# davidcotton/gym-d2d

Hardware: AMD Instinct MI355X
Metric: env agent-steps/sec (batch x agents) (higher is better)
Workload: dtype f32

## Files before the change

### gym_d2d_amd/csrc/d2d_capi.hip

```cpp
#include "../../include/d2d_hip_diag.h"
#include "d2d_internal.h"
#include "d2d_plan.h"

#include <dlfcn.h>

#include <algorithm>
#include <cmath>
#include <cstdio>
#include <cstdlib>
#include <cstring>
#include <exception>
#include <new>
#include <stdexcept>
#include <string>
#include <vector>

namespace {

thread_local std::string g_last_error;

int fail(int code, const std::string& msg) {
    g_last_error = msg;
    return code;
}
// ... 743 lines not shown
        h->table_per_env = 1;
        h->table_links = n_links;
        h->mode = d2d::PL_TABLE_DB;
        h->have_pl = true; h->tables_dirty = true;
        return D2D_OK;
    }
    const size_t elems = (size_t)n_links * n_links * (per_env ? (size_t)h->B : 1);
    int rc = reserve_gain_table(h, elems);
    if (rc) return rc;
    HIP_TRY(d2d::launch_gain_from_db(pl_db_dev, dtype == D2D_F64, elems, h->gain_table, h->num_cus, h->stream));
    HIP_TRY(hipStreamSynchronize(h->stream));
    h->table_per_env = per_env ? 1 : 0;
    h->table_links = n_links;
    h->mode = d2d::PL_TABLE;
    h->have_pl = true; h->tables_dirty = true;
    return D2D_OK;
} D2D_CATCH

int d2d_set_path_loss_link_table(d2d_handle* h, const double* pl_db, int32_t n_links, int32_t per_env) try {
    if (!h || !pl_db) return fail(D2D_ERR_INVALID, "null argument");
    USE_DEVICE(h);
    if (!h->have_links) return fail(D2D_ERR_STATE, "d2d_set_links first: the table is indexed by its link list");
    if (n_links != h->N || n_links < 1) return fail(D2D_ERR_INVALID, "n_links must be the length of the current link list (" + std::to_string(h->N) + ")");
    const size_t elems = (size_t)n_links * n_links * (per_env ? (size_t)h->B : 1);
    int rc = upload_gain_table(h, pl_db, elems);
    if (rc) return rc;
    h->table_per_env = per_env ? 1 : 0;
    h->table_links = n_links;
    h->mode = d2d::PL_TABLE;
    h->have_pl = true; h->tables_dirty = true;
    return D2D_OK;
} D2D_CATCH

int d2d_set_links(d2d_handle* h, int32_t n_links, const int32_t* tx_dev, const int32_t* rx_dev, const int32_t* link_type) try {
    if (!h) return fail(D2D_ERR_INVALID, "null handle");
    USE_DEVICE(h);
    if (n_links < 0 || n_links > h->Nmax) return fail(D2D_ERR_INVALID, "n_links must be in [0, max_links]");
    if (n_links > 0 && (!tx_dev || !rx_dev || !link_type)) return fail(D2D_ERR_INVALID, "null argument");
    for (int i = 0; i < n_links; ++i) {
        if (tx_dev[i] < 0 || tx_dev[i] >= h->D || rx_dev[i] < 0 || rx_dev[i] >= h->D)
            return fail(D2D_ERR_INVALID, "link " + std::to_string(i) + ": device index out of range");
        if (link_type[i] < D2D_UPLINK || link_type[i] > D2D_SIDELINK)
            return fail(D2D_ERR_INVALID, "link " + std::to_string(i) + ": link_type must be 1, 2 or 3");
    }
    HIP_TRY(hipStreamSynchronize(h->stream));
    h->N = n_links;
    h->host_tx.assign(tx_dev, tx_dev + n_links);
    h->host_rx.assign(rx_dev, rx_dev + n_links);
    h->host_type.assign(link_type, link_type + n_links);
    h->fixed_rb.assign((size_t)n_links, INT32_MIN);
    h->fixed_pwr.assign((size_t)n_links, 0);
    h->n_fixed = 0;
    h->tables_dirty = true;
    h->lpos_dirty = true;
    h->have_links = true;
    if (h->table_links) {
        h->table_links = 0;
        h->live_table = nullptr;
        if (d2d::pl_is_table(h->mode)) h->have_pl = false;
    }
    return D2D_OK;
} D2D_CATCH

int d2d_set_fixed_actions(d2d_handle* h, int32_t n_fixed, const int32_t* link_idx, const int32_t* rb, const int32_t* pwr_dbm) try {
    if (!h) return fail(D2D_ERR_INVALID, "null handle");
    if (!h->have_links) return fail(D2D_ERR_STATE, "d2d_set_links first: fixed actions refer to its link list");
    if (n_fixed < 0 || n_fixed > h->N) return fail(D2D_ERR_INVALID, "n_fixed must be in [0, n_links]");
    if (n_fixed > 0 && (!link_idx || !rb || !pwr_dbm)) return fail(D2D_ERR_INVALID, "null argument");
    std::vector<int> frb((size_t)h->N, INT32_MIN), fpw((size_t)h->N, 0);
    for (int k = 0; k < n_fixed; ++k) {
        const int i = link_idx[k];
        if (i < 0 || i >= h->N) return fail(D2D_ERR_INVALID, "fixed action " + std::to_string(k) + ": link index out of range");
        if (frb[i] != INT32_MIN) return fail(D2D_ERR_INVALID, "fixed action " + std::to_string(k) + ": link listed twice");
        if (rb[k] == INT32_MIN) return fail(D2D_ERR_INVALID, "rb out of range");
        frb[i] = rb[k]; fpw[i] = pwr_dbm[k];
    }
    h->fixed_rb.swap(frb); h->fixed_pwr.swap(fpw);
    h->n_fixed = n_fixed;
    h->tables_dirty = true;
    return D2D_OK;
} D2D_CATCH

int d2d_positions_changed(d2d_handle* h) try {
    if (!h) return fail(D2D_ERR_INVALID, "null handle");
    h->lpos_dirty = true;
    h->have_lo = false;
    return D2D_OK;
} D2D_CATCH

int d2d_set_reward(d2d_handle* h, int32_t reward_fn, float param) try {
    if (!h) return fail(D2D_ERR_INVALID, "null handle");
    USE_DEVICE(h);
    if (reward_fn < D2D_REWARD_NONE || reward_fn > D2D_REWARD_CUE_SINR_SHANNON) return fail(D2D_ERR_INVALID, "unknown reward_fn");
    h->reward_fn = reward_fn; h->reward_param = param;
    return D2D_OK;
} D2D_CATCH

int d2d_set_reward_layout(d2d_handle* h, int32_t layout) try {
    if (!h) return fail(D2D_ERR_INVALID, "null handle");
    if (layout != D2D_REWARD_PER_AGENT && layout != D2D_REWARD_PER_ENV) return fail(D2D_ERR_INVALID, "unknown reward layout");
    h->reward_layout = layout;
    return D2D_OK;
} D2D_CATCH

int d2d_set_obs_dtype(d2d_handle* h, int32_t dtype) try {
    if (!h) return fail(D2D_ERR_INVALID, "null handle");
    if (dtype != D2D_F32 && dtype != D2D_F64) return fail(D2D_ERR_INVALID, "obs dtype must be D2D_F32 or D2D_F64");
    USE_DEVICE(h);
    if ((dtype == D2D_F64) != (h->obs_f64 != 0)) {
        Buffer& bf = h->buf[D2D_BUF_OBS];
        if (bf.ptr && bf.owned) { HIP_TRY(hipStreamSynchronize(h->stream)); HIP_TRY(hipFree(bf.ptr)); bf.ptr = nullptr; bf.bytes = 0; }
    }
    h->obs_f64 = dtype == D2D_F64;
    return D2D_OK;
} D2D_CATCH

int d2d_set_obs_mode(d2d_handle* h, int32_t obs_mode) try {
    if (!h) return fail(D2D_ERR_INVALID, "null handle");
    USE_DEVICE(h);
    if (obs_mode < D2D_OBS_NONE || obs_mode > D2D_OBS_LINEAR) return fail(D2D_ERR_INVALID, "unknown obs_mode");
    h->obs_mode = obs_mode;
    return D2D_OK;
} D2D_CATCH

int d2d_set_export_actions(d2d_handle* h, int32_t enabled) try {
    if (!h) return fail(D2D_ERR_INVALID, "null handle");
    h->export_actions = enabled ? 1 : 0;
    return D2D_OK;
} D2D_CATCH

int d2d_set_bucketing(d2d_handle* h, int32_t enabled) try {
    if (!h) return fail(D2D_ERR_INVALID, "null handle");
    USE_DEVICE(h);
    h->bucketing = enabled ? 1 : 0;
    return D2D_OK;
} D2D_CATCH

#if defined(D2D_STEP_ABLATE) && D2D_STEP_ABLATE
extern "C" int d2d_debug_stamps(d2d_handle* h, void* host, size_t bytes) try {
    if (!h || !h->dbg) return fail(D2D_ERR_STATE, "no stamps: set D2D_TUNE_STEP_ABLATE bit 8192 and step first");
    USE_DEVICE(h);
    HIP_TRY(hipStreamSynchronize(h->stream));
    if (!host || bytes > (size_t)h->B * 16 * 16 * 8) return fail(D2D_ERR_INVALID, "stamps: at most B x 16 waves x 16 stamps x 8 bytes");
    HIP_TRY(hipMemcpy(host, h->dbg, bytes, hipMemcpyDeviceToHost));
    return D2D_OK;
} D2D_CATCH
#endif

int d2d_set_tuning(d2d_handle* h, int32_t key, int32_t value) try {
    if (!h) return fail(D2D_ERR_INVALID, "null handle");
    USE_DEVICE(h);
#if !(defined(D2D_DIAG) && D2D_DIAG)
    const bool diag_key = key == D2D_TUNE_OBS_VARIANT || key == D2D_TUNE_OBS_STAGGER || key == D2D_TUNE_STEP_ABLATE;
    const bool diag_value = (key == D2D_TUNE_OBS_NONTEMPORAL && value > 1) || (key == D2D_TUNE_STEP_WALK && value == 1);
    if ((diag_key && value != 0) || diag_value)
        return fail(D2D_ERR_UNSUPPORTED, "this tuning key / value needs the diagnostic build (D2D_BUILD_DIAG=1 python -m gym_d2d_amd.build; include/d2d_hip_diag.h)");
#endif
    switch (key) {
        case D2D_TUNE_OBS_ROWS_PER_WG: h->tune_obs.rows = value; break;
        case D2D_TUNE_OBS_NONTEMPORAL:
            if (value < 0 || value > 5) return fail(D2D_ERR_INVALID, "obs store policy must be in [0, 5]");
            h->tune_obs.nt = value;
            break;
        case D2D_TUNE_OBS_XCD_REMAP: h->tune_obs.xcd = value < 0 ? 0 : value; break;
        case D2D_TUNE_OBS_VARIANT: h->tune_obs.variant = value; break;
        case D2D_TUNE_OBS_STAGGER:
            if (value < 0 || value > 64) return fail(D2D_ERR_INVALID, "stagger must be in [0, 64]");
            h->tune_obs.stagger = value;
            break;
        case D2D_TUNE_STEP_THREADS:
            if (value != 0 && (value < 64 || value > 1024 || value % 64)) return fail(D2D_ERR_INVALID, "threads must be a multiple of 64 in [64,1024]");
            h->tune_step.threads = value;
            break;
        case D2D_TUNE_OBS_BLOCK:
            if (value != 0 && (value < 64 || value > 1024 || value % 64)) return fail(D2D_ERR_INVALID, "block must be a multiple of 64 in [64,1024]");
            h->tune_obs.block = value;
            break;
        case D2D_TUNE_STEP_ENVS_PER_WG:
            if (value < 0 || value > 16) return fail(D2D_ERR_INVALID, "envs per workgroup must be in [0,16]");
            h->tune_step.epw = value;
            break;
        case D2D_TUNE_STEP_BLOCK:
            if (value != 0 && (value < 64 || value > 1024 || value % 64)) return fail(D2D_ERR_INVALID, "block must be a multiple of 64 in [64,1024]");
            h->tune_step.block = value;
            break;
        case D2D_TUNE_STEP_PREFETCH:
            if (value < -1) return fail(D2D_ERR_INVALID, "prefetch distance must be >= -1");
            h->tune_step.prefetch = value;
            break;
        case D2D_TUNE_STEP_LPT:
            if (value != -1 && value != 1 && value != 2) return fail(D2D_ERR_INVALID, "links per thread must be -1 (auto), 1 or 2");
            h->tune_step.lpt = value;
            break;
        case D2D_TUNE_STEP_WALK:
            if (value < -1 || value > 2) return fail(D2D_ERR_INVALID, "walk must be -1, 0, 1 or 2");
            h->tune_step.walk = value;
            break;
        case D2D_TUNE_STEP_ABLATE:
#if defined(D2D_STEP_ABLATE) && D2D_STEP_ABLATE
            h->tune_step.ablate = value;
            break;
#else
            if (value != 0) return fail(D2D_ERR_UNSUPPORTED, "D2D_TUNE_STEP_ABLATE needs the diagnostic build (D2D_BUILD_DIAG=1 python -m gym_d2d_amd.build)");
            break;
#endif
        case D2D_TUNE_STEP_OBS_ROTATE:
            if (value < -1 || value > 65535) return fail(D2D_ERR_INVALID, "obs_rotate must be in [-1, 65535]");
            h->tune_step.obs_rotate = value;
            break;
        case D2D_TUNE_STEP_NT_RESULTS:
            if (value < -1 || value > 1) return fail(D2D_ERR_INVALID, "nt_results must be -1, 0 or 1");
            h->tune_step.nt = value;
            break;
        case D2D_TUNE_STEP_SCALAR_RECORDS:
            if (value < -1 || value > 1) return fail(D2D_ERR_INVALID, "scalar_records must be -1, 0 or 1");
            h->tune_step.srec = value;
            break;
        case D2D_TUNE_STEP_FUSE_OBS:
            if (value < -1 || value > 1) return fail(D2D_ERR_INVALID, "fuse_obs must be -1, 0 or 1");
            h->tune_step.fuse = value;
            break;
        default: return fail(D2D_ERR_INVALID, "unknown tuning key");
    }
    return D2D_OK;
} D2D_CATCH

int d2d_get_buffer(d2d_handle* h, int32_t which, void** dev_ptr, size_t* bytes) try {
    if (!h || !dev_ptr) return fail(D2D_ERR_INVALID, "null argument");
    USE_DEVICE(h);
    if (which < 0 || which >= D2D_BUF_COUNT) return fail(D2D_ERR_INVALID, "unknown buffer");
    if (which == D2D_BUF_OBS && h->N == 0) return fail(D2D_ERR_STATE, "set links before asking for the obs buffer");
    int rc;
    if (which == D2D_BUF_LINK_POS) {
        if (!h->have_links || !h->have_pos) return fail(D2D_ERR_STATE, "link positions need d2d_set_links and positions first");
        rc = refresh_tables(h);
        if (rc) return rc;
        void *px = nullptr, *py = nullptr;
        rc = ensure_buffer(h, D2D_BUF_POS_X, &px);
        if (rc) return rc;
        rc = ensure_buffer(h, D2D_BUF_POS_Y, &py);
        if (rc) return rc;
        rc = refresh_link_positions(h, static_cast<const float*>(px), static_cast<const float*>(py));
        if (rc) return rc;
    }
    rc = ensure_buffer(h, which, dev_ptr);
    if (rc) return rc;
    if (bytes) *bytes = active_bytes(h, which, h->N ? h->N : h->Nmax);
    return D2D_OK;
} D2D_CATCH

int d2d_bind_buffer(d2d_handle* h, int32_t which, void* dev_ptr, size_t bytes) try {
    if (!h) return fail(D2D_ERR_INVALID, "null handle");
    USE_DEVICE(h);
    if (which < 0 || which >= D2D_BUF_COUNT) return fail(D2D_ERR_INVALID, "unknown buffer");
    if (which == D2D_BUF_LINK_POS) return fail(D2D_ERR_INVALID, "D2D_BUF_LINK_POS is derived from POS_X / POS_Y by the library: read-only");
    Buffer& bf = h->buf[which];
    HIP_TRY(hipStreamSynchronize(h->stream));
    if (bf.ptr && bf.owned) HIP_TRY(hipFree(bf.ptr));
    bf.ptr = dev_ptr; bf.bytes = dev_ptr ? bytes : 0; bf.owned = false;
    if (which == D2D_BUF_POS_X || which == D2D_BUF_POS_Y) {
        h->have_pos = h->buf[D2D_BUF_POS_X].ptr && h->buf[D2D_BUF_POS_Y].ptr;
        h->lpos_dirty = true;
        h->have_lo = false;
    }
    return D2D_OK;
} D2D_CATCH

int d2d_upload(d2d_handle* h, int32_t which, const void* host_src, size_t bytes, size_t dst_offset) try {
    if (!h || !host_src) return fail(D2D_ERR_INVALID, "null argument");
    USE_DEVICE(h);
    if (which < 0 || which >= D2D_BUF_COUNT) return fail(D2D_ERR_INVALID, "unknown buffer");
    if (which == D2D_BUF_LINK_POS) return fail(D2D_ERR_INVALID, "D2D_BUF_LINK_POS is derived from POS_X / POS_Y by the library: read-only");
    void* p = nullptr;
    int rc = ensure_buffer(h, which, &p);
    if (rc) return rc;
    if (dst_offset + bytes > h->buf[which].bytes) return fail(D2D_ERR_INVALID, "upload out of range");
    HIP_TRY(hipMemcpyAsync(static_cast<char*>(p) + dst_offset, host_src, bytes, hipMemcpyHostToDevice, h->stream));
    HIP_TRY(hipStreamSynchronize(h->stream));
    if (which == D2D_BUF_POS_X || which == D2D_BUF_POS_Y) {
        h->have_pos = h->buf[D2D_BUF_POS_X].ptr && h->buf[D2D_BUF_POS_Y].ptr;
        h->lpos_dirty = true;
        h->have_lo = false;
    }
    return D2D_OK;
} D2D_CATCH

int d2d_download(d2d_handle* h, int32_t which, void* host_dst, size_t bytes, size_t src_offset) try {
    if (!h || !host_dst) return fail(D2D_ERR_INVALID, "null argument");
    USE_DEVICE(h);
    if (which < 0 || which >= D2D_BUF_COUNT) return fail(D2D_ERR_INVALID, "unknown buffer");
    Buffer bf = h->buf[which];
    if (which == D2D_BUF_LINK_POS) {
        size_t n = 0;
        int rc = d2d_get_buffer(h, which, &bf.ptr, &n);
        if (rc) return rc;
        bf.bytes = n;
    }
    if (!bf.ptr) return fail(D2D_ERR_STATE, "buffer has never been written");
    if (src_offset + bytes > bf.bytes) return fail(D2D_ERR_INVALID, "download out of range");
    HIP_TRY(hipMemcpyAsync(host_dst, static_cast<const char*>(bf.ptr) + src_offset, bytes, hipMemcpyDeviceToHost, h->stream));
    HIP_TRY(hipStreamSynchronize(h->stream));
    return D2D_OK;
} D2D_CATCH

int d2d_set_positions(d2d_handle* h, const float* x, const float* y, int32_t env_begin, int32_t env_count) try {
    if (!h || !x || !y) return fail(D2D_ERR_INVALID, "null argument");
    if (env_begin < 0 || env_count < 0 || env_begin + env_count > h->B) return fail(D2D_ERR_INVALID, "env range out of bounds");
    const size_t off = (size_t)env_begin * h->D * 4, bytes = (size_t)env_count * h->D * 4;
    const bool keep_lo = h->have_lo && env_count < h->B;
    int rc = d2d_upload(h, D2D_BUF_POS_X, x, bytes, off);
    if (rc) return rc;
    rc = d2d_upload(h, D2D_BUF_POS_Y, y, bytes, off);
    if (rc) return rc;
    if (keep_lo) {
// ... 294 lines not shown
```

### gym_d2d_amd/csrc/d2d_internal.h

```cpp
#pragma once
#include <hip/hip_runtime.h>
#include <stdint.h>

namespace d2d {

enum PlMode : int {
    PL_INV_SQUARE = 0,
    PL_POWER = 1,
    PL_TABLE = 2,
    PL_SHADOW = 3,
    PL_POWK = 4,
    PL_TABLE_DB = 5
};

__host__ __device__ constexpr bool pl_is_table(int mode) { return mode == PL_TABLE || mode == PL_TABLE_DB; }

#define D2D_REC_TXDEV_MASK 0x00FFFFFF
#define D2D_REC_TYPE_SHIFT 24
#define D2D_REC_TYPE_MASK 0xF
#define D2D_REC_FIXED_BIT (1 << 28)

#define OPT_LISTS 1
#define OPT_SREC 2
#define OPT_NT 4
#define OPT_PAD 8
#define OPT_XPOS 16

#define LDS_HEAD_BYTES 80u
struct StepLds {
    unsigned aux, rx, sinr, sh, expo, tflat, mask, lists, pool, env_bytes;
    unsigned lo;
};

struct StepArgs {
    int B, N, R, D;
    int mask_words;
    int lpt;
    int rollout;
    StepLds lds;
    int action_mode;
    int act_stride;
    int col_mode;
    int n_fixed;
    int tpe;
    unsigned tpe_magic;
    float inv_n;
    int epw;
    int prefetch_envs;
    int walk;
    int reward_fn;
    float reward_param;
    int write_table;
    int pow_k;
    int rec_uniform;
    int nt_results;
    int ablate;
    unsigned long long* dbg;
    int fuse_obs;
    int obs_rotate;
    unsigned obs_q_per_row;
    unsigned long long obs_q_magic;
    const int* actions;
    const int* rb_in;
    const int* pwr_in;
    const int4* rec_a;
    const float4* rec_b;
    const float4* rec_c;
    const float2* rec_h;
    const int* rec_grp;
    const int* act_cols;
    const unsigned* side_words;
    const float4* lpos;
    const float4* lpos_lo;
    const float* gain_table;
    long long table_env_stride;
    int table_by_link;
    int table_pitch;
    float shadow_chi;
    float shadow_d0sq;
    unsigned shadow_seed_lo, shadow_seed_hi, shadow_step;
    unsigned long long env_offset;
    int* rb_out;
    int* pwr_out;
    float* sinr_db;
    float* snr_db;
    float* rate;
    float* cap;
    float* reward;
    float* reward_env;
    float* table;
    float* obs;
    int* env_flags;
};

struct ObsArgs {
    int B, N;
    int rows_per_wg;
    int chunks;
    int vec;
    unsigned q_per_row;
    unsigned long long q_magic;
    int xcd_remap;
    int nontemporal;
    int block;
    int variant;
    int out_f64;
    int stagger;
    const float* table;
    float* obs;
};

struct StepPlan;
hipError_t launch_step(const StepArgs& a, const StepPlan& p, hipStream_t stream);
hipError_t launch_rollout(const StepArgs& a, const StepPlan& p, hipStream_t stream);
hipError_t launch_obs_expand(const ObsArgs& a, hipStream_t stream);
hipError_t launch_flags_or(const int* env_flags, int B, unsigned* status, hipStream_t stream);
hipError_t launch_link_positions(const float* pos_x, const float* pos_y, const float* lo_x, const float* lo_y, const int4* rec_a,
                                 int B, int N, int D, float4* lpos, float4* lpos_lo, hipStream_t stream);
hipError_t launch_gain_from_db(const void* pl_db, int is_f64, size_t elems, float* gain, int num_cus, hipStream_t stream);
hipError_t launch_reset(int B, int D, int C, float cell_radius, float d2d_radius, unsigned long long seed,
                        unsigned long long episode, unsigned long long env_offset, const unsigned char* fixed_mask,
                        const float* fixed_xy, float* pos_x, float* pos_y, float4* lpos, int N, hipStream_t stream);
hipError_t launch_reset_masked(int B, int D, int C, float cell_radius, float d2d_radius, unsigned long long seed,
                               unsigned long long env_offset, const unsigned char* fixed_mask, const float* fixed_xy, float* pos_x,
                               float* pos_y, float4* lpos, int N, const int* pending, const unsigned* episode, float* lo_x, float* lo_y,
                               const int4* rec_a, float4* rows, float4* rows_lo, hipStream_t stream);

}
```

### gym_d2d_amd/csrc/d2d_obs.hip

```cpp
#include "d2d_internal.h"
#include "d2d_store.h"

namespace d2d {

__device__ __forceinline__ unsigned src_col(unsigned f, unsigned i) {
    const unsigned head = 6u * i;
    return f < 6u ? head + f : (f < head + 6u ? f - 6u : f);
}

template <int VEC, int NT>
__global__ __launch_bounds__(1024) void obs_expand_kernel(const ObsArgs a) {
    extern __shared__ __align__(16) float t_flat[];
    const unsigned N = a.N, tid = threadIdx.x, T = blockDim.x;
    unsigned env, chunk;
    if (a.xcd_remap) {
        const unsigned bid = blockIdx.x, lane8 = bid & 7u, rest = bid >> 3, G = (unsigned)a.xcd_remap;
        const unsigned per_group = a.chunks * G, group = rest / per_group, within = rest % per_group;
        chunk = within / G;
        env = (group * G + within % G) * 8u + lane8;
    } else {
        env = blockIdx.x / a.chunks;
        chunk = blockIdx.x % a.chunks;
    }
    const unsigned row_floats = 6u * N;

    {
        const f32x2* src = reinterpret_cast<const f32x2*>(a.table + (size_t)env * row_floats);
        f32x2* dst = reinterpret_cast<f32x2*>(t_flat);
        for (unsigned k = tid; k < row_floats / 2; k += T) dst[k] = src[k];
    }
    __syncthreads();

    const unsigned r0 = chunk * a.rows_per_wg;
    const unsigned r1 = min(r0 + (unsigned)a.rows_per_wg, N);
    const unsigned q_per_row = a.q_per_row;
    const unsigned total = (r1 - r0) * q_per_row;
    float* out = a.obs + ((size_t)env * N + r0) * row_floats;
    if (a.stagger > 0) {
        const int n = (int)(tid >> 6) * a.stagger;
        for (int k = 0; k < n; ++k) __builtin_amdgcn_s_sleep(1);
    }

    if (VEC == 4 && q_per_row == T) {
        const unsigned f0 = tid * 4u, f1 = f0 + 2u;
        const unsigned t0 = f0 / 6u, t1 = f1 / 6u;
        const bool own0 = f0 < 6u, own1 = f1 < 6u;
        f32x4* o4 = reinterpret_cast<f32x4*>(out) + tid;
        const f32x2* t2 = reinterpret_cast<const f32x2*>(t_flat);
        const auto row = [&](unsigned i) {
            const unsigned head = 6u * i;
            const unsigned s0 = own0 ? head + f0 : (i >= t0 ? f0 - 6u : f0);
            const unsigned s1 = own1 ? head + f1 : (i >= t1 ? f1 - 6u : f1);
            const f32x2 lo = t2[s0 >> 1], hi = t2[s1 >> 1];
            const f32x4 v = {lo.x, lo.y, hi.x, hi.y};
            return v;
        };
        unsigned i = r0;
        for (; i + 1u < r1; i += 2u) {
            const f32x4 va = row(i), vb = row(i + 1u);
            store16<NT>(o4 + (size_t)(i - r0) * T, va);
            store16<NT>(o4 + (size_t)(i + 1u - r0) * T, vb);
        }
        if (i < r1) store16<NT>(o4 + (size_t)(i - r0) * T, row(i));
        return;
    }
#pragma unroll 4
    for (unsigned idx = tid; idx < total; idx += T) {
        const unsigned lr = (unsigned)(((unsigned long long)idx * a.q_magic) >> 40);
        const unsigned q = idx - lr * q_per_row;
        const unsigned i = r0 + lr;
        const unsigned f = q * VEC;
        if (VEC == 4) {
            const f32x2 lo = reinterpret_cast<const f32x2*>(t_flat)[src_col(f, i) >> 1];
            const f32x2 hi = reinterpret_cast<const f32x2*>(t_flat)[src_col(f + 2u, i) >> 1];
            const f32x4 v = {lo.x, lo.y, hi.x, hi.y};
            store16<NT>(reinterpret_cast<f32x4*>(out + (size_t)idx * 4), v);
        } else {
            const f32x2 v = reinterpret_cast<const f32x2*>(t_flat)[src_col(f, i) >> 1];
            f32x2* p = reinterpret_cast<f32x2*>(out + (size_t)idx * 2);
            if (NT) __builtin_nontemporal_store(v, p); else *p = v;
        }
    }
}

template <int NT>
__global__ __launch_bounds__(1024) void obs_expand_flat_kernel(const ObsArgs a) {
    extern __shared__ __align__(16) float t_flat[];
    const unsigned N = a.N, tid = threadIdx.x, T = blockDim.x;
    unsigned env, chunk;
    if (a.xcd_remap) {
        const unsigned bid = blockIdx.x, lane8 = bid & 7u, rest = bid >> 3;
        chunk = rest % a.chunks; env = (rest / a.chunks) * 8u + lane8;
    } else {
        env = blockIdx.x / a.chunks; chunk = blockIdx.x % a.chunks;
    }
    const unsigned row_floats = 6u * N, q_per_row = a.q_per_row, total = N * q_per_row;
    {
        const f32x2* src = reinterpret_cast<const f32x2*>(a.table + (size_t)env * row_floats);
        f32x2* dst = reinterpret_cast<f32x2*>(t_flat);
        for (unsigned k = tid; k < row_floats / 2; k += T) dst[k] = src[k];
    }
    __syncthreads();
    if (a.stagger > 0) {
        const int n = (int)(tid >> 6) * a.stagger;
        for (int k = 0; k < n; ++k) __builtin_amdgcn_s_sleep(1);
    }
    const f32x2* t2 = reinterpret_cast<const f32x2*>(t_flat);
    f32x4* out = reinterpret_cast<f32x4*>(a.obs + (size_t)env * N * row_floats);
    const unsigned base = chunk * (unsigned)a.rows_per_wg * T;
    f32x4 v[4];
    unsigned idx[4];
#pragma unroll
    for (int p = 0; p < 4; ++p) {
        idx[p] = base + (unsigned)p * T + tid;
        if (p < a.rows_per_wg && idx[p] < total) {
            const unsigned i = (unsigned)(((unsigned long long)idx[p] * a.q_magic) >> 40), q = idx[p] - i * q_per_row;
            const unsigned f = q * 4u;
            const f32x2 lo = t2[src_col(f, i) >> 1], hi = t2[src_col(f + 2u, i) >> 1];
            v[p] = f32x4{lo.x, lo.y, hi.x, hi.y};
        }
    }
#pragma unroll
    for (int p = 0; p < 4; ++p)
        if (p < a.rows_per_wg && idx[p] < total) store16<NT>(out + idx[p], v[p]);
}

template <bool NT>
__global__ __launch_bounds__(1024) void obs_expand_f64_kernel(const ObsArgs a) {
    extern __shared__ __align__(16) float t_flat[];
    typedef double f64x2 __attribute__((ext_vector_type(2)));
    const unsigned N = a.N, tid = threadIdx.x, T = blockDim.x;
    unsigned env, chunk;
    if (a.xcd_remap) {
        const unsigned bid = blockIdx.x, lane8 = bid & 7u, rest = bid >> 3, G = (unsigned)a.xcd_remap;
        const unsigned per_group = a.chunks * G, group = rest / per_group, within = rest % per_group;
        chunk = within / G;
        env = (group * G + within % G) * 8u + lane8;
    } else {
        env = blockIdx.x / a.chunks;
        chunk = blockIdx.x % a.chunks;
    }
    const unsigned row_floats = 6u * N, q2 = row_floats / 2u;
    {
        const f32x2* src = reinterpret_cast<const f32x2*>(a.table + (size_t)env * row_floats);
        f32x2* dst = reinterpret_cast<f32x2*>(t_flat);
        for (unsigned k = tid; k < q2; k += T) dst[k] = src[k];
    }
    __syncthreads();
    const unsigned r0 = chunk * a.rows_per_wg;
    const unsigned r1 = min(r0 + (unsigned)a.rows_per_wg, N);
    const f32x2* t2 = reinterpret_cast<const f32x2*>(t_flat);
    double* out = reinterpret_cast<double*>(a.obs) + ((size_t)env * N + r0) * row_floats;
    for (unsigned i = r0; i < r1; ++i) {
        const unsigned head = 6u * i;
        f64x2* o = reinterpret_cast<f64x2*>(out + (size_t)(i - r0) * row_floats);
#pragma unroll 2
        for (unsigned c = tid; c < q2; c += T) {
            const unsigned f = 2u * c;
            const f32x2 v = t2[src_col(f, i) >> 1];
            const f64x2 d = {(double)v.x, (double)v.y};
            if (NT) __builtin_nontemporal_store(d, o + c); else o[c] = d;
        }
        (void)head;
    }
}

template <int NT>
__global__ __launch_bounds__(1024) void obs_expand_flat_f64_kernel(const ObsArgs a) {
    extern __shared__ __align__(16) float t_flat[];
    typedef double f64x2 __attribute__((ext_vector_type(2)));
    const unsigned N = a.N, tid = threadIdx.x, T = blockDim.x;
    unsigned env, chunk;
    if (a.xcd_remap) {
        const unsigned bid = blockIdx.x, lane8 = bid & 7u, rest = bid >> 3;
        chunk = rest % a.chunks; env = (rest / a.chunks) * 8u + lane8;
    } else {
        env = blockIdx.x / a.chunks; chunk = blockIdx.x % a.chunks;
    }
    const unsigned row_floats = 6u * N, q_per_row = a.q_per_row, total = N * q_per_row;
    {
        const f32x2* src = reinterpret_cast<const f32x2*>(a.table + (size_t)env * row_floats);
        f32x2* dst = reinterpret_cast<f32x2*>(t_flat);
        for (unsigned k = tid; k < row_floats / 2; k += T) dst[k] = src[k];
    }
    __syncthreads();
    const f32x2* t2 = reinterpret_cast<const f32x2*>(t_flat);
    f64x2* out = reinterpret_cast<f64x2*>(reinterpret_cast<double*>(a.obs) + (size_t)env * N * row_floats);
    const unsigned base = chunk * (unsigned)a.rows_per_wg * T;
    f32x2 v[4];
    unsigned idx[4];
#pragma unroll
    for (int p = 0; p < 4; ++p) {
        idx[p] = base + (unsigned)p * T + tid;
        if (p < a.rows_per_wg && idx[p] < total) {
            const unsigned i = (unsigned)(((unsigned long long)idx[p] * a.q_magic) >> 40), c = idx[p] - i * q_per_row;
            v[p] = t2[src_col(2u * c, i) >> 1];
        }
    }
#pragma unroll
    for (int p = 0; p < 4; ++p)
        if (p < a.rows_per_wg && idx[p] < total) {
            const f64x2 d = {(double)v[p].x, (double)v[p].y};
            if (NT) __builtin_nontemporal_store(d, out + idx[p]); else out[idx[p]] = d;
        }
}

__global__ __launch_bounds__(1024) void obs_expand_direct_kernel(const ObsArgs a) {
    const unsigned N = a.N, tid = threadIdx.x, T = blockDim.x;
    unsigned env, chunk;
    if (a.xcd_remap) {
        const unsigned bid = blockIdx.x, lane8 = bid & 7u, rest = bid >> 3;
        chunk = rest % a.chunks;
        env = (rest / a.chunks) * 8u + lane8;
    } else {
        env = blockIdx.x / a.chunks;
        chunk = blockIdx.x % a.chunks;
    }
    const unsigned row_floats = 6u * N;
    const float* t_flat = a.table + (size_t)env * row_floats;
    const unsigned r0 = chunk * a.rows_per_wg;
    const unsigned r1 = min(r0 + (unsigned)a.rows_per_wg, N);
    const unsigned q_per_row = a.q_per_row;
    const unsigned total = (r1 - r0) * q_per_row;
    float* out = a.obs + ((size_t)env * N + r0) * row_floats;
#pragma unroll 2
    for (unsigned idx = tid; idx < total; idx += T) {
        const unsigned lr = (unsigned)(((unsigned long long)idx * a.q_magic) >> 40);
        const unsigned q = idx - lr * q_per_row;
        const unsigned i = r0 + lr;
        const unsigned f = q * 4u;
        const f32x2 lo = reinterpret_cast<const f32x2*>(t_flat)[src_col(f, i) >> 1];
        const f32x2 hi = reinterpret_cast<const f32x2*>(t_flat)[src_col(f + 2u, i) >> 1];
        const f32x4 v = {lo.x, lo.y, hi.x, hi.y};
        __builtin_nontemporal_store(v, reinterpret_cast<f32x4*>(out + (size_t)idx * 4));
    }
}

hipError_t launch_obs_expand(const ObsArgs& a, hipStream_t stream) {
    const size_t lds = (size_t)a.N * 6 * sizeof(float);
    dim3 grid((unsigned)a.B * (unsigned)a.chunks), block(a.block > 0 ? a.block : 256);
    if (a.out_f64) {
        if (a.variant == 2 && a.rows_per_wg <= 4) {
            if (a.nontemporal) hipLaunchKernelGGL((obs_expand_flat_f64_kernel<1>), grid, block, lds, stream, a);
            else hipLaunchKernelGGL((obs_expand_flat_f64_kernel<0>), grid, block, lds, stream, a);
        } else if (a.nontemporal) hipLaunchKernelGGL(obs_expand_f64_kernel<true>, grid, block, lds, stream, a);
        else hipLaunchKernelGGL(obs_expand_f64_kernel<false>, grid, block, lds, stream, a);
        return hipGetLastError();
    }
    if (a.variant == 1 && a.vec == 4) {
        hipLaunchKernelGGL(obs_expand_direct_kernel, grid, block, 0, stream, a);
        return hipGetLastError();
    }
    if (a.variant == 2 && a.vec == 4 && a.rows_per_wg <= 4) {
        switch (a.nontemporal) {
            case 0: hipLaunchKernelGGL((obs_expand_flat_kernel<0>), grid, block, lds, stream, a); break;
            case 2: hipLaunchKernelGGL((obs_expand_flat_kernel<2>), grid, block, lds, stream, a); break;
            case 3: hipLaunchKernelGGL((obs_expand_flat_kernel<3>), grid, block, lds, stream, a); break;
            case 4: hipLaunchKernelGGL((obs_expand_flat_kernel<4>), grid, block, lds, stream, a); break;
            case 5: hipLaunchKernelGGL((obs_expand_flat_kernel<5>), grid, block, lds, stream, a); break;
            default: hipLaunchKernelGGL((obs_expand_flat_kernel<1>), grid, block, lds, stream, a); break;
        }
        return hipGetLastError();
    }
    if (a.vec == 4) {
        switch (a.nontemporal) {
            case 0: hipLaunchKernelGGL((obs_expand_kernel<4, 0>), grid, block, lds, stream, a); break;
            case 2: hipLaunchKernelGGL((obs_expand_kernel<4, 2>), grid, block, lds, stream, a); break;
            case 3: hipLaunchKernelGGL((obs_expand_kernel<4, 3>), grid, block, lds, stream, a); break;
            case 4: hipLaunchKernelGGL((obs_expand_kernel<4, 4>), grid, block, lds, stream, a); break;
            case 5: hipLaunchKernelGGL((obs_expand_kernel<4, 5>), grid, block, lds, stream, a); break;
            default: hipLaunchKernelGGL((obs_expand_kernel<4, 1>), grid, block, lds, stream, a); break;
        }
    } else {
        if (a.nontemporal) hipLaunchKernelGGL((obs_expand_kernel<2, 1>), grid, block, lds, stream, a);
        else hipLaunchKernelGGL((obs_expand_kernel<2, 0>), grid, block, lds, stream, a);
    }
    return hipGetLastError();
}

}
```

### gym_d2d_amd/csrc/d2d_plan.h

```cpp
#pragma once
#include "d2d_internal.h"

namespace d2d {

struct StepTuning {
    int threads = 0;
    int epw = 0;
    int block = 0;
    int fuse = -1;
    int walk = -1;
    int prefetch = -1;
    int lpt = -1;
    int nt = -1;
    int srec = -1;
    int obs_rotate = -1;
    int ablate = 0;
};

struct ObsTuning {
    int rows = 0, nt = 1, xcd = 1, block = 0, variant = 0, stagger = 0;
};

struct StepInputs {
    int B, N, R, num_cus;
    int action_mode;
    int n_fixed, col_mode, reward_fn;
    PlMode mode;
    int obs_mode, obs_f64, bucketing;
    int rec_uniform, rec_uniform128;
    int xpos;
    StepTuning tune;
};

struct StepKernel {
    int rollout;
    int mode, lpt, full, hot, opt;
};

struct StepPlan {
    int lpt, tpe;
    unsigned tpe_magic;
    int epw, mask_words, walk, fuse_obs, obs_rotate;
    unsigned obs_q_per_row;
    unsigned long long obs_q_magic;
    StepLds lds;
    int rollout, rec_uniform, nt_results, prefetch_envs;
    unsigned grid;
    int block;
    size_t lds_bytes;
    StepKernel kernel;
    int obs_expand;
};

int plan_step(const StepInputs& in, StepPlan* out, const char** error);
ObsArgs plan_obs(const ObsTuning& t, int B, int N, int out_f64);

}
```

### gym_d2d_amd/csrc/d2d_plan.hip

```cpp
#include "../../include/d2d_hip.h"
#include "d2d_plan.h"

#include <cstring>

namespace d2d {

namespace {

StepLds step_lds_layout(int N, int R, int mask_words, int fuse_obs, int lpt, int reward_fn, int mode, int lists, int xpos) {
    StepLds l;
    std::memset(&l, 0, sizeof(l));
    const unsigned NL = (unsigned)N + (lists ? 1u : 0u);
    unsigned off = LDS_HEAD_BYTES + NL * 16u;
    l.aux = off; off += (unsigned)N * 4u;
    l.rx = off; if (lpt == 0) off += (unsigned)N * 8u;
    l.sinr = off; l.sh = off + (unsigned)N * 4u; if (reward_fn >= 2) off += (unsigned)N * 8u;
    off = (off + 7u) & ~7u;
    l.expo = off; if (mode == PL_POWER || mode == PL_SHADOW || mode == PL_POWK) off += NL * 8u;
    off = (off + 7u) & ~7u;
    l.lo = off; if (xpos) off += NL * 8u;
    l.tflat = off; if (fuse_obs) off += (unsigned)N * 24u;
    off = (off + 15u) & ~15u;
    l.mask = off;
    if (mask_words > 0) off += ((unsigned)R * mask_words + mask_words + (unsigned)R) * 4u;
    off = (off + 15u) & ~15u;
    l.lists = off;
    if (lists) off += (unsigned)R * 16u + (((unsigned)R + 3u) & ~3u) * 4u;
    l.env_bytes = (off + 15u) & ~15u;
    return l;
}

StepLds rollout_lds_layout(int N, int R, int mode, int reward_fn, int xpos) {
    StepLds l;
    std::memset(&l, 0, sizeof(l));
    unsigned off = LDS_HEAD_BYTES + ((unsigned)N + 1u) * 16u;
    l.expo = off;
    if (mode == PL_POWER) off += ((unsigned)N + 1u) * 8u;
    else if (mode == PL_POWK) off += (((unsigned)N + 1u) * 4u + 7u) & ~7u;
    l.lo = off; if (xpos) off += ((unsigned)N + 1u) * 8u;
    off = (off + 15u) & ~15u;
    l.lists = off; off += ((unsigned)R + 1u) * 16u + (((unsigned)R + 1u + 3u) & ~3u) * 4u;
    l.pool = off; off += (unsigned)N * 8u;
    off = (off + 15u) & ~15u;
    l.aux = off; off += 64u;
    l.rx = off;
    if (reward_fn == D2D_REWARD_CUE_SINR_SHANNON) off += ((unsigned)N + 1u) * 4u;
    l.env_bytes = (off + 15u) & ~15u;
    return l;
}

int threads_for(int N, int lpt) { return (((N + lpt - 1) / lpt + 63) / 64) * 64; }

}

int plan_step(const StepInputs& in, StepPlan* out, const char** error) {
    const int N = in.N, R = in.R;
    const StepTuning& t = in.tune;
    if ((size_t)in.B * (size_t)N * 24 >= (1ull << 32)) {
        *error = "envs x links per GPU must stay below 2^32 / 24 (32-bit byte offsets in the step kernel)";
        return D2D_ERR_UNSUPPORTED;
    }
    const bool power_law = in.mode == PL_INV_SQUARE || in.mode == PL_POWER || in.mode == PL_POWK;
    const bool cue_sinr = in.reward_fn == D2D_REWARD_CUE_SINR_SHANNON;
    const bool rec_uniform = in.rec_uniform && t.srec != 0;

    const bool fuse = in.obs_mode == D2D_OBS_LINEAR && !in.obs_f64 && (t.fuse >= 0 ? t.fuse != 0 : N <= 128);
    const int fuse_obs = fuse ? ((6 * N) % 4 == 0 ? 4 : 2) : 0;

    const bool rollout_cfg = in.action_mode == 0 && (in.n_fixed == 0 || (in.n_fixed < N && in.col_mode == 0)) && in.bucketing &&
                             (in.reward_fn == D2D_REWARD_SYSTEM_CAPACITY || in.reward_fn == D2D_REWARD_SHANNON || cue_sinr) &&
                             !fuse && power_law && (t.ablate & ~8192) == 0 && t.prefetch != 0 && t.threads == 0 && t.epw <= 1 &&
                             t.block == 0 && (N % 64 == 0 || N > 64) && N <= 1024;
    const bool lists_can_help = (long long)N <= 4ll * R;
    const bool lists_pay = lists_can_help && (N > 1024 || in.obs_mode == D2D_OBS_NONE || rollout_cfg);
    const int walk_asked = t.walk >= 0 ? t.walk : (lists_pay ? 2 : 0);
    const bool rollout_wanted = in.bucketing && walk_asked == 2 && rollout_cfg && in.col_mode == 0;

    int lpt, tpe;
    if (t.threads > 0) {
        tpe = t.threads;
        lpt = N <= tpe ? 1 : (N <= 2 * tpe ? 2 : 0);
    } else {
        const int want = t.lpt > 0 ? t.lpt : 1;
        lpt = threads_for(N, want) <= 1024 ? want : (threads_for(N, 2) <= 1024 ? 2 : 0);
        tpe = lpt ? threads_for(N, lpt) : 1024;
    }
    const bool lists_asked = in.bucketing && walk_asked == 2 && lpt > 0 && !cue_sinr;
    const auto env_bytes = [&](int W, int lists) { return step_lds_layout(N, R, W, fuse_obs, lpt, in.reward_fn, in.mode, lists, in.xpos).env_bytes; };
    const int words = (N + 31) / 32;
    const int W = in.bucketing && lpt > 0 && N <= 1024 && env_bytes(words, lists_asked) <= 96 * 1024 ? words : 0;
    const bool lists_instead = W == 0 && !lists_asked && lists_can_help && t.walk < 0 && in.bucketing && lpt > 0 && !cue_sinr;
    const bool lists = (lists_asked || lists_instead) && env_bytes(W, 1) <= 96 * 1024;
    const int walk = lists ? 2 : (lists_asked || lists_instead || (walk_asked == 2 && !rollout_wanted)) ? 0 : walk_asked;

    const bool two_asked = (t.lpt > 0 ? t.lpt == 2 : in.rec_uniform128 && rec_uniform && in.mode == PL_INV_SQUARE) && N % 128 == 0;
    const int ro_lpt = two_asked && in.n_fixed == 0 && !cue_sinr && !in.xpos ? 2 : 1;
    const StepLds ro_lds = rollout_lds_layout(N, R, in.mode, in.reward_fn, in.xpos);
    const bool rollout = rollout_wanted && ro_lds.env_bytes <= 64 * 1024;

    StepPlan& p = *out;
    std::memset(&p, 0, sizeof(p));
    p.rollout = rollout;
    p.walk = walk;
    p.fuse_obs = fuse_obs;
    p.lpt = rollout ? ro_lpt : lpt;
    p.tpe = rollout ? threads_for(N, ro_lpt) : tpe;
    p.mask_words = rollout ? 0 : W;
    p.lds = rollout ? ro_lds : step_lds_layout(N, R, W, fuse_obs, lpt, in.reward_fn, in.mode, lists, in.xpos);
    p.rec_uniform = rollout_wanted ? rec_uniform && in.n_fixed == 0 && (!two_asked || in.rec_uniform128) : rec_uniform;
    p.nt_results = in.obs_mode != D2D_OBS_LINEAR && (t.nt > 0 || (rollout && t.nt < 0));
    const size_t env_lds = p.lds.env_bytes;
    if (env_lds > 160 * 1024) {
        *error = "links per env exceed the LDS staging capacity";
        return D2D_ERR_UNSUPPORTED;
    }
    int epw = rollout ? 1 : (t.epw > 0 ? t.epw : (p.tpe >= 256 ? 1 : 256 / p.tpe));
    if (epw > in.B) epw = in.B;
    while (epw > 1 && ((size_t)epw * env_lds > 64 * 1024 || epw * p.tpe > 1024)) --epw;
    p.epw = epw;
    const int threads = epw * p.tpe;
    p.block = t.block > 0 ? (t.block > threads ? t.block : threads) : (fuse && threads < 256 ? 256 : threads);
    if (p.block > 1024) {
        *error = "step workgroup exceeds 1024 threads";
        return D2D_ERR_INVALID;
    }
    int per_cu = (int)((160 * 1024) / ((size_t)epw * env_lds ? (size_t)epw * env_lds : 1));
    if (per_cu > 2048 / p.block) per_cu = 2048 / p.block;
    if (per_cu < 1) per_cu = 1;
    const int dist = t.prefetch >= 0 ? t.prefetch : per_cu * in.num_cus * epw;
    p.prefetch_envs = dist - dist % (8 * epw);
    p.tpe_magic = ((1u << 20) + (unsigned)p.tpe - 1) / (unsigned)p.tpe;
    if (fuse) {
        p.obs_rotate = t.obs_rotate >= 0 ? t.obs_rotate : 29;
        p.obs_q_per_row = (unsigned)(6 * N / fuse_obs);
        p.obs_q_magic = ((1ull << 40) + p.obs_q_per_row - 1) / p.obs_q_per_row;
    }
    p.grid = (unsigned)((in.B + epw - 1) / epw);
    p.lds_bytes = env_lds * (size_t)epw;
    p.obs_expand = in.obs_mode == D2D_OBS_LINEAR && !fuse;

    StepKernel& k = p.kernel;
    k.mode = in.mode;
    k.rollout = rollout;
    const int nt = p.nt_results ? OPT_NT : 0, srec = p.rec_uniform ? OPT_SREC : 0, xp = in.xpos ? OPT_XPOS : 0;
    if (rollout) {
        k.lpt = ro_lpt;
        k.opt = (N % 64 ? nt | OPT_PAD : srec | nt) | xp;
        return D2D_OK;
    }
    const bool full = lpt > 0 && epw == 1 && N == lpt * p.tpe && p.block == p.tpe && !fuse;
    const bool hot_common = power_law && in.action_mode == 0 && in.col_mode == 0 && in.reward_fn == D2D_REWARD_SYSTEM_CAPACITY &&
                            p.prefetch_envs > 0 && (t.ablate & 8191) == 0 && W > 0 && !in.xpos;
    const bool hot1 = hot_common && in.n_fixed == 0 && (walk == 0 || lists) && lpt == 1 && full;
    const bool hot2 = hot_common && in.n_fixed < N && walk == 0 && fuse_obs == 4 && lpt == 1 && !full;
    k.lpt = lpt;
    k.full = full;
    k.hot = hot1 ? 1 : (hot2 ? 2 : 0);
    k.opt = hot1 ? srec | nt : (hot2 ? 0 : (lists ? OPT_LISTS : 0) | xp);
    return D2D_OK;
}

ObsArgs plan_obs(const ObsTuning& t, int B, int N, int out_f64) {
    ObsArgs o;
    std::memset(&o, 0, sizeof(o));
    o.B = B; o.N = N;
    o.out_f64 = out_f64;
    if (out_f64 && t.variant != 3) {
        o.vec = 2;
        o.q_per_row = (unsigned)(3 * N);
        o.q_magic = ((1ull << 40) + o.q_per_row - 1) / o.q_per_row;
        o.block = t.block > 0 ? t.block : 1024;
        int passes = t.rows > 0 ? t.rows : 2;
        if (passes > 4) passes = 4;
        o.rows_per_wg = passes;
        const unsigned total = (unsigned)N * o.q_per_row, slab = (unsigned)passes * (unsigned)o.block;
        o.chunks = (int)((total + slab - 1) / slab);
        o.xcd_remap = (t.xcd > 0 && B % 8 == 0) ? 1 : 0;
        o.nontemporal = t.nt;
        o.variant = 2;
        return o;
    }
    o.vec = (6 * N) % 4 == 0 ? 4 : 2;
    o.q_per_row = (unsigned)(6 * N / o.vec);
    o.q_magic = ((1ull << 40) + o.q_per_row - 1) / o.q_per_row;
    const bool flat = o.vec == 4 && (t.variant == 0 || t.variant == 2) && !out_f64;
    int block = t.block;
    if (block <= 0) {
        block = flat ? 1024 : (int)((o.q_per_row + 63) / 64) * 64;
        if (block < 256) block = 256;
        if (block > 1024) block = 1024;
    }
    int rows = t.rows;
    if (rows <= 0) {
        rows = flat ? 2 : (int)((2u * (unsigned)block + o.q_per_row / 2) / o.q_per_row);
        if (rows < 1) rows = 1;
    }
    if (rows > N && !flat) rows = N;
    o.rows_per_wg = rows;
    o.chunks = (N + rows - 1) / rows;
    if (flat) {
        if (rows > 4) rows = 4;
        o.rows_per_wg = rows;
        const unsigned total = (unsigned)N * o.q_per_row, slab = (unsigned)rows * (unsigned)block;
        o.chunks = (int)((total + slab - 1) / slab);
    }
    o.xcd_remap = (t.xcd > 0 && B % (8 * t.xcd) == 0) ? t.xcd : 0;
    o.nontemporal = t.nt;
    o.block = block;
    o.variant = flat ? 2 : (t.variant == 2 ? 0 : t.variant);
    o.stagger = t.stagger;
    return o;
}

}
```

Baseline: 575.3 million.

## Restructure flat obs expand: staged 16B table loads, magic chunk divide, store policy

Rewrites the flat obs-expansion kernels so the per-env table is staged into LDS with 16-byte loads that are issued before the output-index math. Output indices are precomputed as LDS byte offsets, and the block-to-env divide uses a magic multiply instead of a runtime modulo. The pass count is now a compile-time template parameter, which removes per-pass runtime checks. A new default store policy (-1) lets the planner pick nontemporal mode 5 for small one-trip layouts, at the cost of more kernel instantiations and added complexity.

Measured after the change: 585.6 million, median of 6. 1.02x the previous value.

```diff
diff --git a/gym_d2d_amd/csrc/d2d_capi.hip b/gym_d2d_amd/csrc/d2d_capi.hip
--- a/gym_d2d_amd/csrc/d2d_capi.hip
+++ b/gym_d2d_amd/csrc/d2d_capi.hip
@@ -919,14 +919,14 @@
     USE_DEVICE(h);
 #if !(defined(D2D_DIAG) && D2D_DIAG)
     const bool diag_key = key == D2D_TUNE_OBS_VARIANT || key == D2D_TUNE_OBS_STAGGER || key == D2D_TUNE_STEP_ABLATE;
-    const bool diag_value = (key == D2D_TUNE_OBS_NONTEMPORAL && value > 1) || (key == D2D_TUNE_STEP_WALK && value == 1);
+    const bool diag_value = (key == D2D_TUNE_OBS_NONTEMPORAL && value > 1 && value != 5) || (key == D2D_TUNE_STEP_WALK && value == 1);
     if ((diag_key && value != 0) || diag_value)
         return fail(D2D_ERR_UNSUPPORTED, "this tuning key / value needs the diagnostic build (D2D_BUILD_DIAG=1 python -m gym_d2d_amd.build; include/d2d_hip_diag.h)");
 #endif
     switch (key) {
         case D2D_TUNE_OBS_ROWS_PER_WG: h->tune_obs.rows = value; break;
         case D2D_TUNE_OBS_NONTEMPORAL:
-            if (value < 0 || value > 5) return fail(D2D_ERR_INVALID, "obs store policy must be in [0, 5]");
+            if (value < -1 || value > 5) return fail(D2D_ERR_INVALID, "obs store policy must be in [0, 5], or -1 for the planner's choice");
             h->tune_obs.nt = value;
             break;
         case D2D_TUNE_OBS_XCD_REMAP: h->tune_obs.xcd = value < 0 ? 0 : value; break;
diff --git a/gym_d2d_amd/csrc/d2d_internal.h b/gym_d2d_amd/csrc/d2d_internal.h
--- a/gym_d2d_amd/csrc/d2d_internal.h
+++ b/gym_d2d_amd/csrc/d2d_internal.h
@@ -106,6 +106,7 @@
     int variant;
     int out_f64;
     int stagger;
+    unsigned long long chunk_magic;
     const float* table;
     float* obs;
 };
diff --git a/gym_d2d_amd/csrc/d2d_obs.hip b/gym_d2d_amd/csrc/d2d_obs.hip
--- a/gym_d2d_amd/csrc/d2d_obs.hip
+++ b/gym_d2d_amd/csrc/d2d_obs.hip
@@ -6,6 +6,33 @@
 __device__ __forceinline__ unsigned src_col(unsigned f, unsigned i) {
     const unsigned head = 6u * i;
     return f < 6u ? head + f : (f < head + 6u ? f - 6u : f);
+}
+
+struct StagedPieces { f32x4 r[3]; };
+__device__ __forceinline__ void stage_load16(StagedPieces& s, const float* table_env, unsigned n4, unsigned first, unsigned tid, unsigned T) {
+    const f32x4* src = reinterpret_cast<const f32x4*>(table_env);
+#pragma unroll
+    for (unsigned j = 0; j < 3u; ++j)
+        if (first + j * T < n4) s.r[j] = src[min(first + j * T + tid, n4 - 1u)];
+}
+__device__ __forceinline__ void stage_write16(float* t_flat, const StagedPieces& s, unsigned n4, unsigned first, unsigned tid, unsigned T) {
+    f32x4* dst = reinterpret_cast<f32x4*>(t_flat);
+#pragma unroll
+    for (unsigned j = 0; j < 3u; ++j)
+        if (first + j * T + tid < n4) dst[first + j * T + tid] = s.r[j];
+}
+__device__ __forceinline__ void stage_rest16(float* t_flat, const float* table_env, unsigned n4, unsigned tid, unsigned T) {
+    for (unsigned first = 3u * T; first < n4; first += 3u * T) {
+        StagedPieces s;
+        stage_load16(s, table_env, n4, first, tid, T);
+        stage_write16(t_flat, s, n4, first, tid, T);
+    }
+}
+
+__device__ __forceinline__ unsigned src_byte(unsigned f, unsigned i) {
+    const unsigned head = 6u * i;
+    const unsigned behind = f - (f < head + 6u ? 6u : 0u);
+    return (f < 6u ? head + f : behind) * 4u;
 }
 
 template <int VEC, int NT>
@@ -83,46 +110,75 @@
     }
 }
 
+
+struct FlatHead {
+    unsigned env, chunk, T, q_per_row, stagger;
+    unsigned long long q_magic;
+    const float* table;
+    float* obs;
+};
+__device__ __forceinline__ FlatHead flat_head(const ObsArgs& a) {
+    FlatHead h;
+    h.T = blockDim.x; h.q_per_row = a.q_per_row; h.stagger = (unsigned)a.stagger; h.q_magic = a.q_magic; h.table = a.table; h.obs = a.obs;
+    unsigned chunks = (unsigned)a.chunks, remap = (unsigned)a.xcd_remap;
+    unsigned long long magic = a.chunk_magic;
+    asm volatile("" : "+s"(h.T), "+s"(h.q_per_row), "+s"(h.stagger), "+s"(h.q_magic), "+s"(h.table), "+s"(h.obs), "+s"(chunks), "+s"(remap), "+s"(magic));
+    const unsigned bid = blockIdx.x, rest = remap ? bid >> 3 : bid;
+    const unsigned e = magic ? (unsigned)(((unsigned long long)rest * magic) >> 40) : rest / chunks;
+    h.chunk = rest - e * chunks;
+    h.env = remap ? e * 8u + (bid & 7u) : e;
+    return h;
+}
+
+template <int NT, int PASSES>
+__device__ __forceinline__ void obs_flat_pieces(const ObsArgs& a, const FlatHead& h, float* t_flat) {
+    const unsigned N = a.N, tid = threadIdx.x, T = h.T, env = h.env, chunk = h.chunk;
+    const unsigned row_floats = 6u * N, q_per_row = h.q_per_row, total = N * q_per_row, n4 = row_floats / 4u;
+    const float* table_env = h.table + (size_t)env * row_floats;
+    StagedPieces st;
+    stage_load16(st, table_env, n4, 0u, tid, T);
+    const unsigned base = chunk * (unsigned)PASSES * T;
+    unsigned idx[PASSES], b0[PASSES], b1[PASSES];
+#pragma unroll
+    for (int p = 0; p < PASSES; ++p) {
+        idx[p] = base + (unsigned)p * T + tid;
+        const unsigned at = min(idx[p], total - 1u);
+        const unsigned i = (unsigned)(((unsigned long long)at * h.q_magic) >> 40), q = at - i * q_per_row;
+        const unsigned f = q * 4u;
+        b0[p] = src_byte(f, i); b1[p] = src_byte(f + 2u, i);
+        asm volatile("" : "+v"(b0[p]), "+v"(b1[p]));
+    }
+    f32x4* out = reinterpret_cast<f32x4*>(h.obs + (size_t)env * N * row_floats);
+    stage_write16(t_flat, st, n4, 0u, tid, T);
+    stage_rest16(t_flat, table_env, n4, tid, T);
+    __builtin_amdgcn_sched_barrier(0);
+    __syncthreads();
+    if (h.stagger > 0) {
+        const int n = (int)((tid >> 6) * h.stagger);
+        for (int k = 0; k < n; ++k) __builtin_amdgcn_s_sleep(1);
+    }
+    const char* lds = reinterpret_cast<const char*>(t_flat);
+    f32x2 lo[PASSES], hi[PASSES];
+#pragma unroll
+    for (int p = 0; p < PASSES; ++p) {
+        lo[p] = *reinterpret_cast<const f32x2*>(lds + b0[p]);
+        hi[p] = *reinterpret_cast<const f32x2*>(lds + b1[p]);
+    }
+#pragma unroll
+    for (int p = 0; p < PASSES; ++p)
+        if (idx[p] < total) store16<NT>(out + idx[p], f32x4{lo[p].x, lo[p].y, hi[p].x, hi[p].y});
+}
+
 template <int NT>
 __global__ __launch_bounds__(1024) void obs_expand_flat_kernel(const ObsArgs a) {
     extern __shared__ __align__(16) float t_flat[];
-    const unsigned N = a.N, tid = threadIdx.x, T = blockDim.x;
-    unsigned env, chunk;
-    if (a.xcd_remap) {
-        const unsigned bid = blockIdx.x, lane8 = bid & 7u, rest = bid >> 3;
-        chunk = rest % a.chunks; env = (rest / a.chunks) * 8u + lane8;
-    } else {
-        env = blockIdx.x / a.chunks; chunk = blockIdx.x % a.chunks;
-    }
-    const unsigned row_floats = 6u * N, q_per_row = a.q_per_row, total = N * q_per_row;
-    {
-        const f32x2* src = reinterpret_cast<const f32x2*>(a.table + (size_t)env * row_floats);
-        f32x2* dst = reinterpret_cast<f32x2*>(t_flat);
-        for (unsigned k = tid; k < row_floats / 2; k += T) dst[k] = src[k];
-    }
-    __syncthreads();
-    if (a.stagger > 0) {
-        const int n = (int)(tid >> 6) * a.stagger;
-        for (int k = 0; k < n; ++k) __builtin_amdgcn_s_sleep(1);
-    }
-    const f32x2* t2 = reinterpret_cast<const f32x2*>(t_flat);
-    f32x4* out = reinterpret_cast<f32x4*>(a.obs + (size_t)env * N * row_floats);
-    const unsigned base = chunk * (unsigned)a.rows_per_wg * T;
-    f32x4 v[4];
-    unsigned idx[4];
-#pragma unroll
-    for (int p = 0; p < 4; ++p) {
-        idx[p] = base + (unsigned)p * T + tid;
-        if (p < a.rows_per_wg && idx[p] < total) {
-            const unsigned i = (unsigned)(((unsigned long long)idx[p] * a.q_magic) >> 40), q = idx[p] - i * q_per_row;
-            const unsigned f = q * 4u;
-            const f32x2 lo = t2[src_col(f, i) >> 1], hi = t2[src_col(f + 2u, i) >> 1];
-            v[p] = f32x4{lo.x, lo.y, hi.x, hi.y};
-        }
-    }
-#pragma unroll
-    for (int p = 0; p < 4; ++p)
-        if (p < a.rows_per_wg && idx[p] < total) store16<NT>(out + idx[p], v[p]);
+    const FlatHead h = flat_head(a);
+    switch (a.rows_per_wg) {
+        case 1: obs_flat_pieces<NT, 1>(a, h, t_flat); break;
+        case 2: obs_flat_pieces<NT, 2>(a, h, t_flat); break;
+        case 3: obs_flat_pieces<NT, 3>(a, h, t_flat); break;
+        default: obs_flat_pieces<NT, 4>(a, h, t_flat); break;
+    }
 }
 
 template <bool NT>
@@ -165,44 +221,59 @@
     }
 }
 
+template <int NT, int PASSES>
+__device__ __forceinline__ void obs_flat_f64_pieces(const ObsArgs& a, const FlatHead& h, float* t_flat) {
+    typedef double f64x2 __attribute__((ext_vector_type(2)));
+    const unsigned N = a.N, tid = threadIdx.x, T = h.T, env = h.env, chunk = h.chunk;
+    const unsigned row_floats = 6u * N, q_per_row = h.q_per_row, total = N * q_per_row;
+    const float* table_env = h.table + (size_t)env * row_floats;
+    const bool wide = (row_floats & 3u) == 0u;
+    const unsigned n4 = row_floats / 4u;
+    StagedPieces st;
+    if (wide) stage_load16(st, table_env, n4, 0u, tid, T);
+    const unsigned base = chunk * (unsigned)PASSES * T;
+    unsigned idx[PASSES], b0[PASSES];
+#pragma unroll
+    for (int p = 0; p < PASSES; ++p) {
+        idx[p] = base + (unsigned)p * T + tid;
+        const unsigned at = min(idx[p], total - 1u);
+        const unsigned i = (unsigned)(((unsigned long long)at * h.q_magic) >> 40), c = at - i * q_per_row;
+        b0[p] = src_byte(2u * c, i);
+        asm volatile("" : "+v"(b0[p]));
+    }
+    f32x4* out = reinterpret_cast<f32x4*>(reinterpret_cast<double*>(h.obs) + (size_t)env * N * row_floats);
+    if (wide) {
+        stage_write16(t_flat, st, n4, 0u, tid, T);
+        stage_rest16(t_flat, table_env, n4, tid, T);
+    } else {
+        const f32x2* src = reinterpret_cast<const f32x2*>(table_env);
+        f32x2* dst = reinterpret_cast<f32x2*>(t_flat);
+        for (unsigned k = tid; k < row_floats / 2; k += T) dst[k] = src[k];
+    }
+    __builtin_amdgcn_sched_barrier(0);
+    __syncthreads();
+    const char* lds = reinterpret_cast<const char*>(t_flat);
+    f32x2 v[PASSES];
+#pragma unroll
+    for (int p = 0; p < PASSES; ++p) v[p] = *reinterpret_cast<const f32x2*>(lds + b0[p]);
+#pragma unroll
+    for (int p = 0; p < PASSES; ++p)
+        if (idx[p] < total) {
+            const f64x2 d = {(double)v[p].x, (double)v[p].y};
+            store16<NT>(out + idx[p], __builtin_bit_cast(f32x4, d));
+        }
+}
+
 template <int NT>
 __global__ __launch_bounds__(1024) void obs_expand_flat_f64_kernel(const ObsArgs a) {
     extern __shared__ __align__(16) float t_flat[];
-    typedef double f64x2 __attribute__((ext_vector_type(2)));
-    const unsigned N = a.N, tid = threadIdx.x, T = blockDim.x;
-    unsigned env, chunk;
-    if (a.xcd_remap) {
-        const unsigned bid = blockIdx.x, lane8 = bid & 7u, rest = bid >> 3;
-        chunk = rest % a.chunks; env = (rest / a.chunks) * 8u + lane8;
-    } else {
-        env = blockIdx.x / a.chunks; chunk = blockIdx.x % a.chunks;
-    }
-    const unsigned row_floats = 6u * N, q_per_row = a.q_per_row, total = N * q_per_row;
-    {
-        const f32x2* src = reinterpret_cast<const f32x2*>(a.table + (size_t)env * row_floats);
-        f32x2* dst = reinterpret_cast<f32x2*>(t_flat);
-        for (unsigned k = tid; k < row_floats / 2; k += T) dst[k] = src[k];
-    }
-    __syncthreads();
-    const f32x2* t2 = reinterpret_cast<const f32x2*>(t_flat);
-    f64x2* out = reinterpret_cast<f64x2*>(reinterpret_cast<double*>(a.obs) + (size_t)env * N * row_floats);
-    const unsigned base = chunk * (unsigned)a.rows_per_wg * T;
-    f32x2 v[4];
-    unsigned idx[4];
-#pragma unroll
-    for (int p = 0; p < 4; ++p) {
-        idx[p] = base + (unsigned)p * T + tid;
-        if (p < a.rows_per_wg && idx[p] < total) {
-            const unsigned i = (unsigned)(((unsigned long long)idx[p] * a.q_magic) >> 40), c = idx[p] - i * q_per_row;
-            v[p] = t2[src_col(2u * c, i) >> 1];
-        }
-    }
-#pragma unroll
-    for (int p = 0; p < 4; ++p)
-        if (p < a.rows_per_wg && idx[p] < total) {
-            const f64x2 d = {(double)v[p].x, (double)v[p].y};
-            if (NT) __builtin_nontemporal_store(d, out + idx[p]); else out[idx[p]] = d;
-        }
+    const FlatHead h = flat_head(a);
+    switch (a.rows_per_wg) {
+        case 1: obs_flat_f64_pieces<NT, 1>(a, h, t_flat); break;
+        case 2: obs_flat_f64_pieces<NT, 2>(a, h, t_flat); break;
+        case 3: obs_flat_f64_pieces<NT, 3>(a, h, t_flat); break;
+        default: obs_flat_f64_pieces<NT, 4>(a, h, t_flat); break;
+    }
 }
 
 __global__ __launch_bounds__(1024) void obs_expand_direct_kernel(const ObsArgs a) {
@@ -241,8 +312,14 @@
     dim3 grid((unsigned)a.B * (unsigned)a.chunks), block(a.block > 0 ? a.block : 256);
     if (a.out_f64) {
         if (a.variant == 2 && a.rows_per_wg <= 4) {
-            if (a.nontemporal) hipLaunchKernelGGL((obs_expand_flat_f64_kernel<1>), grid, block, lds, stream, a);
-            else hipLaunchKernelGGL((obs_expand_flat_f64_kernel<0>), grid, block, lds, stream, a);
+            switch (a.nontemporal) {
+                case 0: hipLaunchKernelGGL((obs_expand_flat_f64_kernel<0>), grid, block, lds, stream, a); break;
+                case 2: hipLaunchKernelGGL((obs_expand_flat_f64_kernel<2>), grid, block, lds, stream, a); break;
+                case 3: hipLaunchKernelGGL((obs_expand_flat_f64_kernel<3>), grid, block, lds, stream, a); break;
+                case 4: hipLaunchKernelGGL((obs_expand_flat_f64_kernel<4>), grid, block, lds, stream, a); break;
+                case 5: hipLaunchKernelGGL((obs_expand_flat_f64_kernel<5>), grid, block, lds, stream, a); break;
+                default: hipLaunchKernelGGL((obs_expand_flat_f64_kernel<1>), grid, block, lds, stream, a); break;
+            }
         } else if (a.nontemporal) hipLaunchKernelGGL(obs_expand_f64_kernel<true>, grid, block, lds, stream, a);
         else hipLaunchKernelGGL(obs_expand_f64_kernel<false>, grid, block, lds, stream, a);
         return hipGetLastError();
diff --git a/gym_d2d_amd/csrc/d2d_plan.h b/gym_d2d_amd/csrc/d2d_plan.h
--- a/gym_d2d_amd/csrc/d2d_plan.h
+++ b/gym_d2d_amd/csrc/d2d_plan.h
@@ -18,7 +18,7 @@
 };
 
 struct ObsTuning {
-    int rows = 0, nt = 1, xcd = 1, block = 0, variant = 0, stagger = 0;
+    int rows = 0, nt = -1, xcd = 1, block = 0, variant = 0, stagger = 0;
 };
 
 struct StepInputs {
diff --git a/gym_d2d_amd/csrc/d2d_plan.hip b/gym_d2d_amd/csrc/d2d_plan.hip
--- a/gym_d2d_amd/csrc/d2d_plan.hip
+++ b/gym_d2d_amd/csrc/d2d_plan.hip
@@ -160,6 +160,17 @@
     return D2D_OK;
 }
 
+namespace {
+
+int obs_store_policy(int nt, bool one_trip, int pieces) { return nt >= 0 ? nt : (one_trip && pieces <= 2 ? 5 : 1); }
+
+unsigned long long obs_chunk_magic(const ObsArgs& o) {
+    const unsigned long long grid = (unsigned long long)o.B * (unsigned)o.chunks, n = o.xcd_remap ? grid / 8 : grid, d = (unsigned)o.chunks;
+    return n < (1ull << 24) && n * d < (1ull << 40) ? ((1ull << 40) + d - 1) / d : 0;
+}
+
+}
+
 ObsArgs plan_obs(const ObsTuning& t, int B, int N, int out_f64) {
     ObsArgs o;
     std::memset(&o, 0, sizeof(o));
@@ -169,6 +180,7 @@
         o.vec = 2;
         o.q_per_row = (unsigned)(3 * N);
         o.q_magic = ((1ull << 40) + o.q_per_row - 1) / o.q_per_row;
+        const bool one_trip = (6 * N) % 4 == 0;
         o.block = t.block > 0 ? t.block : 1024;
         int passes = t.rows > 0 ? t.rows : 2;
         if (passes > 4) passes = 4;
@@ -176,8 +188,9 @@
         const unsigned total = (unsigned)N * o.q_per_row, slab = (unsigned)passes * (unsigned)o.block;
         o.chunks = (int)((total + slab - 1) / slab);
         o.xcd_remap = (t.xcd > 0 && B % 8 == 0) ? 1 : 0;
-        o.nontemporal = t.nt;
+        o.nontemporal = obs_store_policy(t.nt, one_trip, passes);
         o.variant = 2;
+        o.chunk_magic = obs_chunk_magic(o);
         return o;
     }
     o.vec = (6 * N) % 4 == 0 ? 4 : 2;
@@ -205,10 +218,11 @@
         o.chunks = (int)((total + slab - 1) / slab);
     }
     o.xcd_remap = (t.xcd > 0 && B % (8 * t.xcd) == 0) ? t.xcd : 0;
-    o.nontemporal = t.nt;
+    o.nontemporal = obs_store_policy(t.nt, flat, o.rows_per_wg);
     o.block = block;
     o.variant = flat ? 2 : (t.variant == 2 ? 0 : t.variant);
     o.stagger = t.stagger;
+    if (flat) o.chunk_magic = obs_chunk_magic(o);
     return o;
 }
 
```
